# agiresearch/OpenP5

Measured on AMD Instinct MI355X. Metric: train_samples_per_sec, higher is better.
Workload: dtype bf16; 1 GPU; ML-1M-shaped sequential prompts, t5-small V=32100, B=64/GPU L=128 T=8, dropout 0.1, fwd+bwd+clip+AdamW (BASELINE.json configs[1]); global_batch=64, seq_len=128, tgt_len=8, parallelism=dp1

## Files before the change

openp5_amd/csrc/p5_attn.h:

```cpp
#pragma once
#include "p5_device.h"
#include "p5_rng.h"

struct P5AttnArgs {
  const void* Q; const void* K; const void* V;
  void* O;
  float* lse;
  const void* dO;
  void* dQ; void* dK; void* dV;
  float* Dvec;
  const float* rel_table;
  float* d_rel_table;
  const int* bucket_lut;
  int lut_half;
  const int64_t* kmask;
  int B, H, Lq, Lk;
  int ldq, ldk, ldv, ldo, lddo, lddq, lddk, lddv;
  int causal;
  int rel_copies;
  int rel_stride;
  P5Drop drop;
  uint32_t* keep_bits;
  float* dot_out;
};
// ... 992 lines not shown
#pragma unroll
          for (int t = 0; t < 4; ++t) {
            f32x4 sacc = {0.f, 0.f, 0.f, 0.f}, dpacc = {0.f, 0.f, 0.f, 0.f};
            mma16<T>(sacc, ld16(cK + t * 2048 + koff0), qf0);
            mma16<T>(sacc, ld16(cK + t * 2048 + koff1), qf1);
            mma16<T>(dpacc, ld16(cV + t * 2048 + koff0), dof0);
            mma16<T>(dpacc, ld16(cV + t * 2048 + koff1), dof1);
            const int kb = ch * 64 + t * 16 + g * 4;
            const f32x4 kn = *(const f32x4*)(skneg + kb);
            const float* pb = sbias + (kb - qic + a.Lq - 1);
            float mk[4] = {1.f, 1.f, 1.f, 1.f};
            if constexpr (MODE == 1) {
#pragma unroll
              for (int r = 0; r < 4; ++r) mk[r] = (kw[t][r] & lanebit) ? a.drop.scale : 0.f;
            } else if constexpr (MODE == 2) {
#pragma unroll
              for (int r = 0; r < 4; ++r) mk[r] = p5_keep(seed, a.drop.site_key, rowbase + (uint32_t)(kb + r), a.drop.thr) ? a.drop.scale : 0.f;
            }
#pragma unroll
            for (int r = 0; r < 4; ++r) {
              const int kj = kb + r;
              float ex = fmaf(sacc[r], P5_LOG2E, pb[r] + (kn[r] - lse_q));
              if constexpr (!PLAIN) ex = (qok & !(causal & (kj > qi))) ? ex : P5_NEG_INF;
              const float p = p5_exp2(ex);
              dsv[t][r] = p * (dpacc[r] * mk[r] - D_q);
            }
            if (do_rel) st4<T>(pw + li * DSTR + (DPAD + t * 16 + g * 4) * C::SZ, dsv[t]);
          }
        };
        if (use_bits) { if (plain) tiles(AttnBool<true>(), P5EpiTagA<1>()); else tiles(AttnBool<false>(), P5EpiTagA<1>()); }
        else if (do_drop) { if (plain) tiles(AttnBool<true>(), P5EpiTagA<2>()); else tiles(AttnBool<false>(), P5EpiTagA<2>()); }
        else { if (plain) tiles(AttnBool<true>(), P5EpiTagA<0>()); else tiles(AttnBool<false>(), P5EpiTagA<0>()); }
        if (do_rel) {
          P5_WAVE_SYNC();
          float x1 = 0.f, x2 = 0.f;
#pragma unroll
          for (int qr = 0; qr < 16; ++qr) {
            x1 += to_f<T>(*(const T*)(dg1 + qr * (DSTR + 2)));
            x2 += to_f<T>(*(const T*)(dg2 + qr * (DSTR + 2)));
          }
          x2 = lane < 15 ? x2 : 0.f;
          P5_WAVE_SYNC();
          const float y1 = __shfl(x1, src), y2 = __shfl(x2, src);
          R[ch] += up ? y1 : 0.f;
          R[ch + 1] += up ? y2 : y1;
          R[ch + 2] += up ? 0.f : y2;
        }
#pragma unroll
        for (int u = 0; u < 2; ++u) {
          const float d8[8] = {dsv[2 * u][0], dsv[2 * u][1], dsv[2 * u][2], dsv[2 * u][3], dsv[2 * u + 1][0], dsv[2 * u + 1][1], dsv[2 * u + 1][2], dsv[2 * u + 1][3]};
          const u32x4 da = pack16<T>(d8);
#pragma unroll
          for (int dt = 0; dt < 4; ++dt) {
            const char* base = cK + (u * 32 + trow) * 128 + (((dt * 2 + ((li >> 1) & 1)) ^ tsw) << 4) + (li & 1) * 8;
            const u32x2 lo = lds_tr16_b64(base);
            const u32x2 hi = lds_tr16_b64(base + 16 * 128);
            u32x4 kb4;
            kb4[0] = lo[0]; kb4[1] = lo[1]; kb4[2] = hi[0]; kb4[3] = hi[1];
            mma16<T>(dq[dt], da, kb4);
          }
        }
      }
    }
    const float one[4] = {1.f, 1.f, 1.f, 1.f};
    wave_store_16x64<T>((T*)a.dQ + (size_t)b * a.Lq * a.lddq + h * 64, a.lddq, q0, a.Lq, dq, one, pw, lane);
    if (do_rel && q0 + 128 < a.Lq) {
      P5_WAVE_SYNC();
      clear_diag_tile();
    }
    {
      const float t16 = R[16], t17 = R[17];
#pragma unroll
      for (int k = 17; k >= 2; --k) R[k] = R[k - 2];
      R[0] = t16; R[1] = t17;
    }
  }
  if (do_rel) {
    __syncthreads();
    float* rows = (float*)tKV;
    for (int i = lane; i < 1024; i += 64) rows[wave * 1024 + i] = 0.f;
    P5_WAVE_SYNC();
#pragma unroll
    for (int k = 0; k < 18; ++k) {
      int J = (cw - 2 * nblk + k) % 18;
      if (J < 0) J += 18;
      const int idx = 64 * J + lane - 16;
      if (idx >= 0 && idx < nrel) rows[wave * 1024 + idx] = R[k];
    }
    __syncthreads();
    for (int i = tid; i < nrel; i += NT) {
      float t = rows[i];
#pragma unroll
      for (int w = 1; w < 8; ++w) t += rows[w * 1024 + i];
      rows[i] = t;
    }
    __syncthreads();
    rel_bias_grad_flush<512>(a, h, b, rows, sbias, tid);
  }
}

template <int NQT>
__global__ __launch_bounds__(512) void p5_attn_bwd_dkv_head_kernel(P5AttnArgs a) {
  using T = bf16;
  using C = AttnC<T>;
  constexpr int LQ = NQT * 16, NT = 512, NP = LQ * 8 / NT;
  static_assert(NQT == 16 || NQT == 32, "whole-head attention backward: 256 or 512 query slots");
  __shared__ __attribute__((aligned(16))) char tQ[LQ * 128];
  __shared__ __attribute__((aligned(16))) char tDO[LQ * 128];
  __shared__ __attribute__((aligned(16))) char pbuf[8 * 16 * C::TS];
  constexpr int PADB = 64;
  __shared__ float sbias[PADB + 1024];
  __shared__ __attribute__((aligned(16))) float slse[LQ];
  __shared__ __attribute__((aligned(16))) float sD[LQ];

  const int tid = threadIdx.x, lane = tid & 63, wave = tid >> 6, g = lane >> 4, li = lane & 15;
  const int b = blockIdx.x / a.H, h = blockIdx.x % a.H;
  const T* Q = (const T*)a.Q + (size_t)b * a.Lq * a.ldq + h * 64;
  const T* K = (const T*)a.K + (size_t)b * a.Lk * a.ldk + h * 64;
  const T* V = (const T*)a.V + (size_t)b * a.Lk * a.ldv + h * 64;
  const T* dO = (const T*)a.dO + (size_t)b * a.Lq * a.lddo + h * 64;
  const int nrel = a.Lq + a.Lk - 1;
  {
    u32x4 rq[NP], rd[NP];
#pragma unroll
    for (int i = 0; i < NP; ++i) {
      const int p = tid + i * NT, row = p >> 3, pc = p & 7;
      rq[i] = row < a.Lq ? ld16(Q + (size_t)row * a.ldq + pc * 8) : zero16();
    }
#pragma unroll
    for (int i = 0; i < NP; ++i) {
      const int p = tid + i * NT, row = p >> 3, pc = p & 7;
      rd[i] = row < a.Lq ? ld16(dO + (size_t)row * a.lddo + pc * 8) : zero16();
    }
    for (int i = tid; i < PADB + 1023; i += NT) {
      const int j = i - PADB;
      sbias[i] = (a.rel_table && j >= 0 && j < nrel) ? P5_LOG2E * a.rel_table[a.bucket_lut[j - (a.Lq - 1) + a.lut_half] * a.H + h] : 0.f;
    }
    for (int i = tid; i < LQ; i += NT) {
      slse[i] = i < a.Lq ? P5_LOG2E * attn_bwd_row_lse(a.lse[((size_t)b * a.H + h) * a.Lq + i]) : 0.f;
      sD[i] = i < a.Lq ? a.Dvec[((size_t)b * a.H + h) * a.Lq + i] : 0.f;
    }
#pragma unroll
    for (int i = 0; i < NP; ++i) {
      const int p = tid + i * NT, row = p >> 3, pc = p & 7;
      st16(tQ + row * 128 + ((pc ^ ((row >> 1) & 7)) << 4), rq[i]);
      st16(tDO + row * 128 + ((pc ^ ((row >> 1) & 7)) << 4), rd[i]);
    }
  }
  u32x4 kn[2], vn[2];
  bool kok_n;
  {
    const int krow = wave * 16 + li;
#pragma unroll
    for (int c = 0; c < 2; ++c) {
      kn[c] = krow < a.Lk ? ld16(K + (size_t)krow * a.ldk + c * 32 + g * 8) : zero16();
      vn[c] = krow < a.Lk ? ld16(V + (size_t)krow * a.ldv + c * 32 + g * 8) : zero16();
    }
    kok_n = krow < a.Lk && (!a.kmask || a.kmask[(size_t)b * a.Lk + krow] != 0);
  }
  __syncthreads();

  const bool causal = a.causal != 0;
  const bool do_drop = a.drop.state != nullptr && a.drop.thr != 0;
  const bool use_bits = do_drop && a.keep_bits != nullptr;
  const uint32_t seed = p5_seed(a.drop);
  const int ksw = (li >> 1) & 7;
  const int koff0 = li * 128 + (((0 + g) ^ ksw) << 4), koff1 = li * 128 + (((4 + g) ^ ksw) << 4);
  const int trow = g * 4 + (li >> 2), tsw = (g * 2 + (li >> 3)) & 7;
  char* pw = pbuf + wave * 16 * C::TS;
  const int nqc = (a.Lq + 63) / 64;
  for (int k0 = wave * 16; k0 < a.Lk; k0 += 128) {
    const u32x4 kf0 = kn[0], kf1 = kn[1], vf0 = vn[0], vf1 = vn[1];
    const bool kok = kok_n;
    const int kj = k0 + li;
    if (k0 + 128 < a.Lk) {
      const int krow = k0 + 128 + li;
#pragma unroll
      for (int c = 0; c < 2; ++c) {
        kn[c] = krow < a.Lk ? ld16(K + (size_t)krow * a.ldk + c * 32 + g * 8) : zero16();
        vn[c] = krow < a.Lk ? ld16(V + (size_t)krow * a.ldv + c * 32 + g * 8) : zero16();
      }
      kok_n = krow < a.Lk && (!a.kmask || a.kmask[(size_t)b * a.Lk + krow] != 0);
    }
    const uint32_t headbase = (uint32_t)((((size_t)b * a.H + h) * a.Lq) * a.Lk) + (uint32_t)kj;
    const char* kpk = use_bits ? (const char*)(a.keep_bits + ((size_t)b * a.H + h) * ((a.Lq + 15) / 16) * 256) +
                                     ((((kj >> 3) & 1) * 128 + (kj >> 4) * 4 + (kj & 3)) * 4 + ((kj >> 2) & 1) * 2) : nullptr;
    f32x4 dk[4], dv[4];
#pragma unroll
    for (int dt = 0; dt < 4; ++dt) { dk[dt] = (f32x4){0.f, 0.f, 0.f, 0.f}; dv[dt] = (f32x4){0.f, 0.f, 0.f, 0.f}; }
    unsigned pcn[4] = {0u, 0u, 0u, 0u};
    if (use_bits) {
#pragma unroll
      for (int t = 0; t < 4; ++t) pcn[t] = t * 16 < a.Lq ? *(const unsigned short*)(kpk + (size_t)t * 1024) : 0u;
    }
    for (int qc = 0; qc < nqc; ++qc) {
      const char* cQ = tQ + qc * 64 * 128;
      const char* cD = tDO + qc * 64 * 128;
      float pv[4][4], dsv[4][4];
      const unsigned pcc[4] = {pcn[0], pcn[1], pcn[2], pcn[3]};
      if (use_bits && (qc + 1) * 64 < a.Lq) {
#pragma unroll
        for (int t = 0; t < 4; ++t) pcn[t] = ((qc + 1) * 4 + t) * 16 < a.Lq ? *(const unsigned short*)(kpk + (size_t)((qc + 1) * 4 + t) * 1024) : 0u;
      }
      const bool plain = !causal && (qc + 1) * 64 <= a.Lq;
      auto tiles = [&](auto plain_c, auto mode_c) {
        constexpr bool PLAIN = decltype(plain_c)::value;
        constexpr int MODE = decltype(mode_c)::value;
#pragma unroll
        for (int t = 0; t < 4; ++t) {
          f32x4 sacc = {0.f, 0.f, 0.f, 0.f}, dpacc = {0.f, 0.f, 0.f, 0.f};
          mma16<T>(sacc, ld16(cQ + t * 2048 + koff0), kf0);
          mma16<T>(sacc, ld16(cQ + t * 2048 + koff1), kf1);
          mma16<T>(dpacc, ld16(cD + t * 2048 + koff0), vf0);
          mma16<T>(dpacc, ld16(cD + t * 2048 + koff1), vf1);
          const int qb = qc * 64 + t * 16 + g * 4;
          const f32x4 ls = *(const f32x4*)(slse + qb), dd = *(const f32x4*)(sD + qb);
          const float* pbq = sbias + (PADB + kj - qb + a.Lq - 4);
          const float bias[4] = {pbq[3], pbq[2], pbq[1], pbq[0]};
          const uint32_t tbase = headbase + (uint32_t)qb * (uint32_t)a.Lk;
          float mk[4] = {1.f, 1.f, 1.f, 1.f};
          if constexpr (MODE == 1) {
            const unsigned piece = pcc[t] >> (g * 4);
#pragma unroll
            for (int r = 0; r < 4; ++r) mk[r] = ((piece >> r) & 1u) ? a.drop.scale : 0.f;
          } else if constexpr (MODE == 2) {
#pragma unroll
            for (int r = 0; r < 4; ++r) mk[r] = p5_keep(seed, a.drop.site_key, tbase + (uint32_t)r * (uint32_t)a.Lk, a.drop.thr) ? a.drop.scale : 0.f;
          }
#pragma unroll
          for (int r = 0; r < 4; ++r) {
            const int qi = qb + r;
            const bool ok = PLAIN ? kok : (kok & (qi < a.Lq) & !(causal & (kj > qi)));
            float ex = fmaf(sacc[r], P5_LOG2E, bias[r] - ls[r]);
            ex = ok ? ex : P5_NEG_INF;
            const float p = p5_exp2(ex);
            pv[t][r] = p * mk[r];
            dsv[t][r] = p * (dpacc[r] * mk[r] - dd[r]);
          }
        }
      };
      if (use_bits) { if (plain) tiles(AttnBool<true>(), P5EpiTagA<1>()); else tiles(AttnBool<false>(), P5EpiTagA<1>()); }
      else if (do_drop) { if (plain) tiles(AttnBool<true>(), P5EpiTagA<2>()); else tiles(AttnBool<false>(), P5EpiTagA<2>()); }
      else { if (plain) tiles(AttnBool<true>(), P5EpiTagA<0>()); else tiles(AttnBool<false>(), P5EpiTagA<0>()); }
#pragma unroll
      for (int u = 0; u < 2; ++u) {
        const float p8[8] = {pv[2 * u][0], pv[2 * u][1], pv[2 * u][2], pv[2 * u][3], pv[2 * u + 1][0], pv[2 * u + 1][1], pv[2 * u + 1][2], pv[2 * u + 1][3]};
        const float d8[8] = {dsv[2 * u][0], dsv[2 * u][1], dsv[2 * u][2], dsv[2 * u][3], dsv[2 * u + 1][0], dsv[2 * u + 1][1], dsv[2 * u + 1][2], dsv[2 * u + 1][3]};
        const u32x4 pa = pack16<T>(p8), sa = pack16<T>(d8);
#pragma unroll
        for (int dt = 0; dt < 4; ++dt) {
          const int off = (u * 32 + trow) * 128 + (((dt * 2 + ((li >> 1) & 1)) ^ tsw) << 4) + (li & 1) * 8;
          u32x2 lo = lds_tr16_b64(cD + off), hi = lds_tr16_b64(cD + off + 16 * 128);
          u32x4 f;
          f[0] = lo[0]; f[1] = lo[1]; f[2] = hi[0]; f[3] = hi[1];
          mma16<T>(dv[dt], pa, f);
          lo = lds_tr16_b64(cQ + off);
          hi = lds_tr16_b64(cQ + off + 16 * 128);
          f[0] = lo[0]; f[1] = lo[1]; f[2] = hi[0]; f[3] = hi[1];
          mma16<T>(dk[dt], sa, f);
        }
      }
    }
    const float one[4] = {1.f, 1.f, 1.f, 1.f};
    wave_store_16x64<T>((T*)a.dK + (size_t)b * a.Lk * a.lddk + h * 64, a.lddk, k0, a.Lk, dk, one, pw, lane);
    wave_store_16x64<T>((T*)a.dV + (size_t)b * a.Lk * a.lddv + h * 64, a.lddv, k0, a.Lk, dv, one, pw, lane);
  }
}

#ifdef P5_EMU
#define P5_ATTN_SMALL_OCC
#else
#define P5_ATTN_SMALL_OCC __attribute__((amdgpu_waves_per_eu(2, 2)))
#endif
template <class T>
__global__ __launch_bounds__(256) P5_ATTN_SMALL_OCC void p5_attn_bwd_small_kernel(P5AttnArgs a) {
  using C = AttnC<T>;
  constexpr int KR = C::KCH;
  constexpr int RS = 64 + 16;
    __shared__ __attribute__((aligned(16))) char tileKV[2 * 64 * C::TS];
  char* const tileK = tileKV;
  char* const tileV = tileKV + 64 * C::TS; __shared__ __attribute__((aligned(16))) char tileQ[32 * C::TS];
  __shared__ __attribute__((aligned(16))) char tileDO[32 * C::TS];
  __shared__ __attribute__((aligned(16))) char aP[4][16 * RS];
  __shared__ __attribute__((aligned(16))) char aS[4][16 * RS];
  __shared__ __attribute__((aligned(16))) char bS[4][16 * RS];
  __shared__ __attribute__((aligned(16))) char wscr[4][16 * C::TS];
  static_assert(2 * 64 * C::TS >= 4 * 16 * 68 * 4, "the dQ partial sums reuse the K and V tiles");
  float (*sdq)[16][68] = (float (*)[16][68])tileKV;
  __shared__ __attribute__((aligned(16))) float sbias[1024];
  __shared__ float sdb[4][528];
  __shared__ __attribute__((aligned(16))) float slse[16];
  __shared__ __attribute__((aligned(16))) float sD[16];

  const int tid = threadIdx.x, lane = tid & 63, wave = tid >> 6, g = lane >> 4, li = lane & 15;
  const int b = blockIdx.y / a.H, h = blockIdx.y % a.H;
  const T* Q = (const T*)a.Q + (size_t)b * a.Lq * a.ldq + h * 64;
  const T* K = (const T*)a.K + (size_t)b * a.Lk * a.ldk + h * 64;
  const T* V = (const T*)a.V + (size_t)b * a.Lk * a.ldv + h * 64;
  const T* dO = (const T*)a.dO + (size_t)b * a.Lq * a.lddo + h * 64;
  const T* O = (const T*)a.O + (size_t)b * a.Lq * a.ldo + h * 64;
  const int nrel = a.Lq + a.Lk - 1;
  const int nch = (a.Lk + 63) / 64;

  for (int p = tid; p < 32 * C::PPR; p += 256) {
    const int row = p / C::PPR, pc = p % C::PPR;
    st16(tileQ + row * C::TS + pc * 16, row < a.Lq ? ld16(Q + (size_t)row * a.ldq + pc * C::EPF) : zero16());
    st16(tileDO + row * C::TS + pc * 16, row < a.Lq ? ld16(dO + (size_t)row * a.lddo + pc * C::EPF) : zero16());
  }
  if (a.rel_table) {
    for (int i = tid; i < nrel; i += 256) sbias[i] = a.rel_table[a.bucket_lut[i - (a.Lq - 1) + a.lut_half] * a.H + h];
    if (a.d_rel_table)
      for (int i = tid; i < 4 * 528; i += 256) (&sdb[0][0])[i] = 0.f;
  }
  if (tid < 64) {
    const int q = tid >> 2, part = tid & 3;
    float d = 0.f;
    if (q < a.Lq) {
      for (int c = 0; c < 16; c += C::EPF) {
        float x[8], y[8];
        unpack16<T>(ld16(dO + (size_t)q * a.lddo + part * 16 + c), x);
        unpack16<T>(ld16(O + (size_t)q * a.ldo + part * 16 + c), y);
#pragma unroll
        for (int e = 0; e < C::EPF; ++e) d += x[e] * y[e];
      }
    }
    d += __shfl_xor(d, 1);
    d += __shfl_xor(d, 2);
    if (part == 0) {
      sD[q] = d;
      slse[q] = q < a.Lq ? a.lse[((size_t)b * a.H + h) * a.Lq + q] : 0.f;
      if (a.Dvec && q < a.Lq) a.Dvec[((size_t)b * a.H + h) * a.Lq + q] = d;
    }
  }
  for (int i = lane; i < 16 * RS / 4; i += 64) {
    ((unsigned*)aP[wave])[i] = 0u; ((unsigned*)aS[wave])[i] = 0u; ((unsigned*)bS[wave])[i] = 0u;
  }
  __syncthreads();

  u32x4 qf[C::NCK], dof[C::NCK];
#pragma unroll
  for (int c = 0; c < C::NCK; ++c) { qf[c] = tile_frag_kc<T>(tileQ, 0, c, lane); dof[c] = tile_frag_kc<T>(tileDO, 0, c, lane); }
  const bool causal = a.causal != 0;
  const bool do_drop = a.drop.state != nullptr && a.drop.thr != 0;
  const uint32_t seed = p5_seed(a.drop);
  const int qb = g * 4;
  const f32x4 ls = *(const f32x4*)(slse + qb), dd = *(const f32x4*)(sD + qb);
  const int kc_w = (wave * 16) / KR, koff = (wave * 16) % KR;

  f32x4 dq[4];
#pragma unroll
  for (int dt = 0; dt < 4; ++dt) dq[dt] = (f32x4){0.f, 0.f, 0.f, 0.f};

  for (int ch = 0; ch < nch; ++ch) {
    __syncthreads();
    stage_tile64<T>(tileK, K + (size_t)ch * 64 * a.ldk, a.ldk, a.Lk - ch * 64, tid);
    stage_tile64<T>(tileV, V + (size_t)ch * 64 * a.ldv, a.ldv, a.Lk - ch * 64, tid);
    __syncthreads();
    const int k0 = ch * 64 + wave * 16, kj = k0 + li;
    if (k0 < a.Lk) {
      const bool kok = kj < a.Lk && (!a.kmask || a.kmask[(size_t)b * a.Lk + kj] != 0);
      f32x4 sacc = {0.f, 0.f, 0.f, 0.f}, dpacc = {0.f, 0.f, 0.f, 0.f};
#pragma unroll
      for (int c = 0; c < C::NCK; ++c) {
        mma16<T>(sacc, qf[c], tile_frag_kc<T>(tileK, wave * 16, c, lane));
        mma16<T>(dpacc, dof[c], tile_frag_kc<T>(tileV, wave * 16, c, lane));
      }
      float pv[4], dsv[4];
#pragma unroll
      for (int r = 0; r < 4; ++r) {
        const int qi = qb + r;
        const int qic = qi < a.Lq ? qi : a.Lq - 1;
        const float bias = a.rel_table ? sbias[(kj < a.Lk ? kj : a.Lk - 1) - qic + a.Lq - 1] : 0.f;
        const float mk = do_drop ? (p5_keep(seed, a.drop.site_key, (uint32_t)((((size_t)b * a.H + h) * a.Lq + qic) * a.Lk) + (uint32_t)kj, a.drop.thr) ? a.drop.scale : 0.f) : 1.f;
        const bool ok = kok & (qi < a.Lq) & !(causal & (kj > qi));
        const float p = p5_exp<T>((sacc[r] + bias) - ls[r]);
        pv[r] = ok ? p * mk : 0.f;
        dsv[r] = ok ? p * (dpacc[r] * mk - dd[r]) : 0.f;
      }
      P5_WAVE_SYNC();
      st4<T>(aP[wave] + li * RS + qb * C::SZ, pv);
      st4<T>(aS[wave] + li * RS + qb * C::SZ, dsv);
#pragma unroll
      for (int r = 0; r < 4; ++r) *(T*)(bS[wave] + (qb + r) * RS + (koff + li) * C::SZ) = from_f<T>(dsv[r]);
      P5_WAVE_SYNC();
      if (a.d_rel_table) {
        for (int dg = lane; dg < 31; dg += 64) {
          float sum = 0.f;
#pragma unroll
          for (int qr = 0; qr < 16; ++qr) {
            const int kcol = dg - 15 + qr;
            if (kcol >= 0 && kcol < 16) sum += to_f<T>(*(const T*)(bS[wave] + qr * RS + (koff + kcol) * C::SZ));
          }
          const int idx = k0 + dg - 15 + a.Lq - 1;
          if (idx >= 0 && idx < nrel) sdb[wave][idx] += sum;
        }
      }
      f32x4 dk[4], dv[4];
      const u32x4 pa = ld16(aP[wave] + li * RS + g * 16), sa = ld16(aS[wave] + li * RS + g * 16);
      const u32x4 dsa = ld16(bS[wave] + li * RS + g * 16);
#pragma unroll
      for (int dt = 0; dt < 4; ++dt) {
        dk[dt] = (f32x4){0.f, 0.f, 0.f, 0.f}; dv[dt] = (f32x4){0.f, 0.f, 0.f, 0.f};
        mma16<T>(dv[dt], pa, tile_frag_ks<T>(tileDO, dt * 16, 0, lane));
        mma16<T>(dk[dt], sa, tile_frag_ks<T>(tileQ, dt * 16, 0, lane));
        mma16<T>(dq[dt], dsa, tile_frag_ks<T>(tileK, dt * 16, kc_w, lane));
      }
      const float one[4] = {1.f, 1.f, 1.f, 1.f};
      wave_store_16x64<T>((T*)a.dK + (size_t)b * a.Lk * a.lddk + h * 64, a.lddk, k0, a.Lk, dk, one, wscr[wave], lane);
      wave_store_16x64<T>((T*)a.dV + (size_t)b * a.Lk * a.lddv + h * 64, a.lddv, k0, a.Lk, dv, one, wscr[wave], lane);
    }
  }
  __syncthreads();
#pragma unroll
  for (int dt = 0; dt < 4; ++dt)
#pragma unroll
    for (int r = 0; r < 4; ++r) sdq[wave][g * 4 + r][dt * 16 + li] = dq[dt][r];
  __syncthreads();
  if (wave == 0) {
    f32x4 t[4];
#pragma unroll
    for (int dt = 0; dt < 4; ++dt)
#pragma unroll
      for (int r = 0; r < 4; ++r)
        t[dt][r] = ((sdq[0][g * 4 + r][dt * 16 + li] + sdq[1][g * 4 + r][dt * 16 + li]) + sdq[2][g * 4 + r][dt * 16 + li]) + sdq[3][g * 4 + r][dt * 16 + li];
    const float one[4] = {1.f, 1.f, 1.f, 1.f};
    wave_store_16x64<T>((T*)a.dQ + (size_t)b * a.Lq * a.lddq + h * 64, a.lddq, 0, a.Lq, t, one, wscr[0], lane);
  }
  if (a.d_rel_table) {
    for (int i = tid; i < nrel; i += 256) sdb[0][i] = ((sdb[0][i] + sdb[1][i]) + sdb[2][i]) + sdb[3][i];
    __syncthreads();
    rel_bias_grad_flush<256>(a, h, b, &sdb[0][0], sbias, tid);
  }
}

__device__ static __forceinline__ u32x4 frag_ks_stride(const char* lds, int stride, int e0, int kc, int lane) {
  const int g = lane >> 4, i = lane & 15;
  const char* base = lds + (kc * 32 + g * 8 + (i >> 2)) * stride + (e0 + (i & 3) * 4) * 2;
  const u32x2 lo = lds_tr16_b64(base), hi = lds_tr16_b64(base + 4 * stride);
  u32x4 r;
  r[0] = lo[0]; r[1] = lo[1]; r[2] = hi[0]; r[3] = hi[1];
  return r;
}

template <class T>
__global__ __launch_bounds__(512) void p5_attn_bwd_fused_kernel(P5AttnArgs a) {
  static_assert(sizeof(T) == 2, "fused attention backward: bf16 only");
  using C = AttnC<T>;
  constexpr int TP = 128 * 2 + 16;
  __shared__ __attribute__((aligned(16))) char tK[128 * C::TS];
  __shared__ __attribute__((aligned(16))) char tV[128 * C::TS];
  __shared__ __attribute__((aligned(16))) char tQ[128 * C::TS];
  __shared__ __attribute__((aligned(16))) char tDO[128 * C::TS];
  __shared__ __attribute__((aligned(16))) char mP[128 * TP];
  __shared__ __attribute__((aligned(16))) char mS[128 * TP];
  __shared__ float sbias[256];
  __shared__ float sdiag[8 * 144];
  __shared__ __attribute__((aligned(16))) float skneg[128];

  const int tid = threadIdx.x, lane = tid & 63, wave = tid >> 6, g = lane >> 4, li = lane & 15;
  const int b = blockIdx.x / a.H, h = blockIdx.x % a.H;
  const T* Q = (const T*)a.Q + (size_t)b * a.Lq * a.ldq + h * 64;
  const T* K = (const T*)a.K + (size_t)b * a.Lk * a.ldk + h * 64;
  const T* V = (const T*)a.V + (size_t)b * a.Lk * a.ldv + h * 64;
  const T* dO = (const T*)a.dO + (size_t)b * a.Lq * a.lddo + h * 64;
  const T* O = (const T*)a.O + (size_t)b * a.Lq * a.ldo + h * 64;
  const int nrel = a.Lq + a.Lk - 1;

  u32x4 rq[2], rk[2], rv[2], rdo[2], of[2];
#pragma unroll
  for (int i = 0; i < 2; ++i) {
    const int p = tid + i * 512, row = p >> 3, pc = p & 7;
    rq[i] = row < a.Lq ? ld16(Q + (size_t)row * a.ldq + pc * 8) : zero16();
    rdo[i] = row < a.Lq ? ld16(dO + (size_t)row * a.lddo + pc * 8) : zero16();
    rk[i] = row < a.Lk ? ld16(K + (size_t)row * a.ldk + pc * 8) : zero16();
    rv[i] = row < a.Lk ? ld16(V + (size_t)row * a.ldv + pc * 8) : zero16();
  }
  const int q0 = wave * 16, qi = q0 + li;
  const bool qok = qi < a.Lq;
  const int qic = qok ? qi : a.Lq - 1;
#pragma unroll
  for (int c = 0; c < 2; ++c) of[c] = qok ? ld16(O + (size_t)qi * a.ldo + c * 32 + g * 8) : zero16();
  const float lse_q = qok ? P5_LOG2E * attn_bwd_row_lse(a.lse[((size_t)b * a.H + h) * a.Lq + qi]) : 0.f;
  stage_bias_mask(a, b, h, sbias, skneg, 128, tid, P5_LOG2E, 256);
#pragma unroll
  for (int i = 0; i < 2; ++i) {
    const int p = tid + i * 512, row = p >> 3, pc = p & 7;
    st16(tQ + row * C::TS + pc * 16, rq[i]);
    st16(tDO + row * C::TS + pc * 16, rdo[i]);
    st16(tK + row * C::TS + pc * 16, rk[i]);
    st16(tV + row * C::TS + pc * 16, rv[i]);
  }
  __syncthreads();

  const bool causal = a.causal != 0;
  const bool do_drop = a.drop.state != nullptr && a.drop.thr != 0;
  const uint32_t seed = p5_seed(a.drop);
  const uint32_t rowbase = (uint32_t)((((size_t)b * a.H + h) * a.Lq + qi) * a.Lk);
  u32x4 qf[2], dof[2];
  float D_q = 0.f;
#pragma unroll
  for (int c = 0; c < 2; ++c) {
    qf[c] = tile_frag_kc<T>(tQ, q0, c, lane);
    dof[c] = tile_frag_kc<T>(tDO, q0, c, lane);
    float x[8], y[8];
    unpack16<T>(dof[c], x);
    unpack16<T>(of[c], y);
#pragma unroll
    for (int e = 0; e < 8; ++e) D_q += x[e] * y[e];
  }
  D_q += __shfl_xor(D_q, 16);
  D_q += __shfl_xor(D_q, 32);
  char* myP = mP + qi * TP;
  char* myS = mS + qi * TP;
  const bool plain = !causal && q0 + 16 <= a.Lq;
#pragma unroll
  for (int t = 0; t < 8; ++t) {
    f32x4 sacc = {0.f, 0.f, 0.f, 0.f}, dpacc = {0.f, 0.f, 0.f, 0.f};
#pragma unroll
    for (int c = 0; c < 2; ++c) {
      mma16<T>(sacc, tile_frag_kc<T>(tK, t * 16, c, lane), qf[c]);
      mma16<T>(dpacc, tile_frag_kc<T>(tV, t * 16, c, lane), dof[c]);
    }
    const int kb = t * 16 + g * 4;
    const f32x4 kn = *(const f32x4*)(skneg + kb);
    const float* pb = sbias + (kb - qic + a.Lq - 1);
    float mk[4] = {1.f, 1.f, 1.f, 1.f};
    if (do_drop) {
#pragma unroll
      for (int r = 0; r < 4; ++r) mk[r] = p5_keep(seed, a.drop.site_key, rowbase + (uint32_t)(kb + r), a.drop.thr) ? a.drop.scale : 0.f;
    }
    float pv[4], dsv[4];
#pragma unroll
    for (int r = 0; r < 4; ++r) {
      const int kj = kb + r;
      float ex = fmaf(sacc[r], P5_LOG2E, pb[r] + (kn[r] - lse_q));
      if (!plain) ex = (qok & !(causal & (kj > qi))) ? ex : P5_NEG_INF;
      const float p = p5_exp2(ex);
      pv[r] = p * mk[r];
      dsv[r] = p * (dpacc[r] * mk[r] - D_q);
    }
    st4<T>(myP + kb * 2, pv);
    st4<T>(myS + kb * 2, dsv);
  }
  P5_WAVE_SYNC();
  if (a.d_rel_table) {
    for (int dd = lane; dd < 128 + 15; dd += 64) {
      float sum = 0.f;
#pragma unroll
      for (int qr = 0; qr < 16; ++qr) {
        const int kcol = dd - 15 + qr;
        const bool in = (kcol >= 0) & (kcol < 128);
        const float v = to_f<T>(*(const T*)(mS + (q0 + qr) * TP + (in ? kcol : 0) * 2));
        sum += in ? v : 0.f;
      }
      sdiag[wave * 144 + dd] = sum;
    }
  }
  f32x4 dq[4];
#pragma unroll
  for (int dt = 0; dt < 4; ++dt) dq[dt] = (f32x4){0.f, 0.f, 0.f, 0.f};
#pragma unroll
  for (int kc = 0; kc < 4; ++kc) {
    const u32x4 dsa = ld16(myS + kc * 64 + g * 16);
#pragma unroll
    for (int dt = 0; dt < 4; ++dt) mma16<T>(dq[dt], dsa, tile_frag_ks<T>(tK, dt * 16, kc, lane));
  }
  __syncthreads();

  if (a.d_rel_table) {
    float pv[4];
    int pb[4];
#pragma unroll
    for (int j = 0; j < 4; ++j) {
      const int i = lane + 64 * j;
      float v = 0.f;
      pb[j] = -1;
      if (i < nrel) {
        pb[j] = a.bucket_lut[i - (a.Lq - 1) + a.lut_half] & 63;
#pragma unroll
        for (int w = 0; w < 8; ++w) {
          const int dd = i + 15 + 16 * w - (a.Lq - 1);
          const bool in = (dd >= 0) & (dd < 128 + 15);
          const float x = sdiag[w * 144 + (in ? dd : 0)];
          v += in ? x : 0.f;
        }
      }
      pv[j] = v;
    }
    for (int bk = wave; bk < a.rel_copies; bk += 8) {
      float acc = 0.f;
#pragma unroll
      for (int j = 0; j < 4; ++j) acc += pb[j] == bk ? pv[j] : 0.f;
      acc = wave_sum(acc);
      if (lane == 0) a.d_rel_table[(size_t)b * a.rel_stride + bk * a.H + h] = acc;
    }
  }
  const float one[4] = {1.f, 1.f, 1.f, 1.f};
  char* scratch = tK + wave * 16 * C::TS;
  const bool want_dot = a.dot_out != nullptr;
  float dot[2] = {0.f, 0.f};
  u32x4 fwk[2], fwq[2], fwv[2];
  if (want_dot) {
#pragma unroll
    for (int p = 0; p < 2; ++p) {
      const int off = (wave * 16 + p * 8 + (lane >> 3)) * C::TS + (lane & 7) * 16;
      fwk[p] = ld16(tK + off);
      fwq[p] = ld16(tQ + off);
      fwv[p] = ld16(tV + off);
    }
    wave_store_16x64_dot<T>((T*)a.dQ + (size_t)b * a.Lq * a.lddq + h * 64, a.lddq, q0, a.Lq, dq, scratch, lane, fwq, dot);
  } else {
    wave_store_16x64<T>((T*)a.dQ + (size_t)b * a.Lq * a.lddq + h * 64, a.lddq, q0, a.Lq, dq, one, scratch, lane);
  }

  const int k0 = wave * 16;
  f32x4 dk[4], dv[4];
#pragma unroll
  for (int dt = 0; dt < 4; ++dt) { dk[dt] = (f32x4){0.f, 0.f, 0.f, 0.f}; dv[dt] = (f32x4){0.f, 0.f, 0.f, 0.f}; }
#pragma unroll
  for (int kc = 0; kc < 4; ++kc) {
    const u32x4 pa = frag_ks_stride(mP, TP, k0, kc, lane);
    const u32x4 sa = frag_ks_stride(mS, TP, k0, kc, lane);
#pragma unroll
    for (int dt = 0; dt < 4; ++dt) {
      mma16<T>(dv[dt], pa, tile_frag_ks<T>(tDO, dt * 16, kc, lane));
      mma16<T>(dk[dt], sa, tile_frag_ks<T>(tQ, dt * 16, kc, lane));
    }
  }
  if (want_dot) {
    wave_store_16x64_dot<T>((T*)a.dK + (size_t)b * a.Lk * a.lddk + h * 64, a.lddk, k0, a.Lk, dk, scratch, lane, fwk, dot);
    wave_store_16x64_dot<T>((T*)a.dV + (size_t)b * a.Lk * a.lddv + h * 64, a.lddv, k0, a.Lk, dv, scratch, lane, fwv, dot);
#pragma unroll
    for (int p = 0; p < 2; ++p) {
      float t = dot[p];
      t += __shfl_xor(t, 1);
      t += __shfl_xor(t, 2);
      t += __shfl_xor(t, 4);
      const int tok = wave * 16 + p * 8 + (lane >> 3);
      if ((lane & 7) == 0 && tok < a.Lq) a.dot_out[((size_t)b * a.Lq + tok) * a.H + h] = t;
    }
    return;
  }
  wave_store_16x64<T>((T*)a.dK + (size_t)b * a.Lk * a.lddk + h * 64, a.lddk, k0, a.Lk, dk, one, scratch, lane);
  wave_store_16x64<T>((T*)a.dV + (size_t)b * a.Lk * a.lddv + h * 64, a.lddv, k0, a.Lk, dv, one, scratch, lane);
}
```

Measured before the change: 16250 samples/s.

## Prefetch K/V chunks into registers and batch prologue loads in attention backward

For 16-bit types, the attention backward kernel now issues all prologue global loads (Q, dO, O, lse, bucket LUT, rel bias, first K/V chunk) into registers before any shared-memory stores, using scheduling fences to group them. It also software-pipelines the K/V chunk loop, fetching chunk ch+1 into registers while chunk ch is computed, and reads the key mask together with that fetch. This is meant to hide global-memory latency in a short kernel (Lk=128, few chunks). The cost is higher register pressure, which could lower occupancy.

```diff
diff --git a/openp5_amd/csrc/p5_attn.h b/openp5_amd/csrc/p5_attn.h
--- a/openp5_amd/csrc/p5_attn.h
+++ b/openp5_amd/csrc/p5_attn.h
@@ -1318,34 +1318,133 @@
   const int nrel = a.Lq + a.Lk - 1;
   const int nch = (a.Lk + 63) / 64;
 
-  for (int p = tid; p < 32 * C::PPR; p += 256) {
-    const int row = p / C::PPR, pc = p % C::PPR;
-    st16(tileQ + row * C::TS + pc * 16, row < a.Lq ? ld16(Q + (size_t)row * a.ldq + pc * C::EPF) : zero16());
-    st16(tileDO + row * C::TS + pc * 16, row < a.Lq ? ld16(dO + (size_t)row * a.lddo + pc * C::EPF) : zero16());
-  }
-  if (a.rel_table) {
-    for (int i = tid; i < nrel; i += 256) sbias[i] = a.rel_table[a.bucket_lut[i - (a.Lq - 1) + a.lut_half] * a.H + h];
-    if (a.d_rel_table)
-      for (int i = tid; i < 4 * 528; i += 256) (&sdb[0][0])[i] = 0.f;
-  }
-  if (tid < 64) {
+  constexpr int NPKV = 64 * C::PPR / 256, NREL = 3;
+  constexpr bool PRE = sizeof(T) == 2;
+  u32x4 rk[NPKV], rv[NPKV];
+  const int64_t* const kmp = a.kmask ? a.kmask + (size_t)b * a.Lk : (const int64_t*)a.Q;
+  int64_t rkm = 1;
+  auto kv_fetch = [&](int ch) {
+    const int valid_rows = a.Lk - ch * 64;
+#pragma unroll
+    for (int i = 0; i < NPKV; ++i) {
+      const int p = tid + i * 256, row = p / C::PPR, pc = p % C::PPR;
+      const int rowc = row < valid_rows ? row : valid_rows - 1;
+      rk[i] = ld16(K + ((size_t)ch * 64 + rowc) * a.ldk + pc * C::EPF);
+      rv[i] = ld16(V + ((size_t)ch * 64 + rowc) * a.ldv + pc * C::EPF);
+    }
+    const int kj = ch * 64 + wave * 16 + li;
+    rkm = kmp[(a.kmask && kj < a.Lk) ? kj : 0];
+  };
+  auto kv_publish = [&](int ch) {
+    const int valid_rows = a.Lk - ch * 64;
+#pragma unroll
+    for (int i = 0; i < NPKV; ++i) {
+      const int p = tid + i * 256, row = p / C::PPR, pc = p % C::PPR;
+      st16(tileK + row * C::TS + pc * 16, row < valid_rows ? rk[i] : zero16());
+      st16(tileV + row * C::TS + pc * 16, row < valid_rows ? rv[i] : zero16());
+    }
+  };
+
+  if constexpr (PRE) {
+    constexpr int NQ = 32 * C::PPR / 256, ND = 16 / C::EPF;
+    const bool has_tab = a.rel_table != nullptr;
+    const int* const lutp = has_tab ? a.bucket_lut : (const int*)a.lse;
+    const float* const tab = has_tab ? a.rel_table : a.lse;
+    const int tab_ld = has_tab ? a.H : 0, tab_h = has_tab ? h : 0, lut0 = has_tab ? a.lut_half - (a.Lq - 1) : 0;
+    int lutv[NREL];
+#pragma unroll
+    for (int j = 0; j < NREL; ++j) {
+      const int i = tid + j * 256;
+      lutv[j] = lutp[lut0 + ((has_tab && i < nrel) ? i : 0)];
+    }
+    P5_SCHED_FENCE();
+    kv_fetch(0);
+    u32x4 tq[NQ], tdo[NQ], xd[ND], yo[ND];
+#pragma unroll
+    for (int i = 0; i < NQ; ++i) {
+      const int p = tid + i * 256, row = p / C::PPR, pc = p % C::PPR;
+      const int rowc = row < a.Lq ? row : a.Lq - 1;
+      tq[i] = ld16(Q + (size_t)rowc * a.ldq + pc * C::EPF);
+      tdo[i] = ld16(dO + (size_t)rowc * a.lddo + pc * C::EPF);
+    }
     const int q = tid >> 2, part = tid & 3;
-    float d = 0.f;
-    if (q < a.Lq) {
-      for (int c = 0; c < 16; c += C::EPF) {
-        float x[8], y[8];
-        unpack16<T>(ld16(dO + (size_t)q * a.lddo + part * 16 + c), x);
-        unpack16<T>(ld16(O + (size_t)q * a.ldo + part * 16 + c), y);
-#pragma unroll
-        for (int e = 0; e < C::EPF; ++e) d += x[e] * y[e];
-      }
-    }
-    d += __shfl_xor(d, 1);
-    d += __shfl_xor(d, 2);
-    if (part == 0) {
-      sD[q] = d;
-      slse[q] = q < a.Lq ? a.lse[((size_t)b * a.H + h) * a.Lq + q] : 0.f;
-      if (a.Dvec && q < a.Lq) a.Dvec[((size_t)b * a.H + h) * a.Lq + q] = d;
+    const int qc = q < a.Lq ? q : a.Lq - 1;
+#pragma unroll
+    for (int k = 0; k < ND; ++k) {
+      xd[k] = ld16(dO + (size_t)qc * a.lddo + part * 16 + k * C::EPF);
+      yo[k] = ld16(O + (size_t)qc * a.ldo + part * 16 + k * C::EPF);
+    }
+    const float lse_r = a.lse[((size_t)b * a.H + h) * a.Lq + qc];
+    P5_SCHED_FENCE();
+    float tb[NREL];
+#pragma unroll
+    for (int j = 0; j < NREL; ++j) tb[j] = tab[lutv[j] * tab_ld + tab_h];
+    P5_SCHED_FENCE();
+#pragma unroll
+    for (int i = 0; i < NQ; ++i) {
+      const int p = tid + i * 256, row = p / C::PPR, pc = p % C::PPR;
+      st16(tileQ + row * C::TS + pc * 16, row < a.Lq ? tq[i] : zero16());
+      st16(tileDO + row * C::TS + pc * 16, row < a.Lq ? tdo[i] : zero16());
+    }
+    if (has_tab) {
+#pragma unroll
+      for (int j = 0; j < NREL; ++j) {
+        const int i = tid + j * 256;
+        if (i < nrel) sbias[i] = tb[j];
+      }
+      if (a.d_rel_table)
+        for (int i = tid; i < 4 * 528; i += 256) (&sdb[0][0])[i] = 0.f;
+    }
+    if (tid < 64) {
+      float d = 0.f;
+      if (q < a.Lq) {
+#pragma unroll
+        for (int k = 0; k < ND; ++k) {
+          float x[8], y[8];
+          unpack16<T>(xd[k], x);
+          unpack16<T>(yo[k], y);
+#pragma unroll
+          for (int e = 0; e < C::EPF; ++e) d += x[e] * y[e];
+        }
+      }
+      d += __shfl_xor(d, 1);
+      d += __shfl_xor(d, 2);
+      if (part == 0) {
+        sD[q] = d;
+        slse[q] = q < a.Lq ? lse_r : 0.f;
+        if (a.Dvec && q < a.Lq) a.Dvec[((size_t)b * a.H + h) * a.Lq + q] = d;
+      }
+    }
+  } else {
+    for (int p = tid; p < 32 * C::PPR; p += 256) {
+      const int row = p / C::PPR, pc = p % C::PPR;
+      st16(tileQ + row * C::TS + pc * 16, row < a.Lq ? ld16(Q + (size_t)row * a.ldq + pc * C::EPF) : zero16());
+      st16(tileDO + row * C::TS + pc * 16, row < a.Lq ? ld16(dO + (size_t)row * a.lddo + pc * C::EPF) : zero16());
+    }
+    if (a.rel_table) {
+      for (int i = tid; i < nrel; i += 256) sbias[i] = a.rel_table[a.bucket_lut[i - (a.Lq - 1) + a.lut_half] * a.H + h];
+      if (a.d_rel_table)
+        for (int i = tid; i < 4 * 528; i += 256) (&sdb[0][0])[i] = 0.f;
+    }
+    if (tid < 64) {
+      const int q = tid >> 2, part = tid & 3;
+      float d = 0.f;
+      if (q < a.Lq) {
+        for (int c = 0; c < 16; c += C::EPF) {
+          float x[8], y[8];
+          unpack16<T>(ld16(dO + (size_t)q * a.lddo + part * 16 + c), x);
+          unpack16<T>(ld16(O + (size_t)q * a.ldo + part * 16 + c), y);
+#pragma unroll
+          for (int e = 0; e < C::EPF; ++e) d += x[e] * y[e];
+        }
+      }
+      d += __shfl_xor(d, 1);
+      d += __shfl_xor(d, 2);
+      if (part == 0) {
+        sD[q] = d;
+        slse[q] = q < a.Lq ? a.lse[((size_t)b * a.H + h) * a.Lq + q] : 0.f;
+        if (a.Dvec && q < a.Lq) a.Dvec[((size_t)b * a.H + h) * a.Lq + q] = d;
+      }
     }
   }
   for (int i = lane; i < 16 * RS / 4; i += 64) {
@@ -1369,12 +1468,13 @@
 
   for (int ch = 0; ch < nch; ++ch) {
     __syncthreads();
-    stage_tile64<T>(tileK, K + (size_t)ch * 64 * a.ldk, a.ldk, a.Lk - ch * 64, tid);
-    stage_tile64<T>(tileV, V + (size_t)ch * 64 * a.ldv, a.ldv, a.Lk - ch * 64, tid);
+    if constexpr (!PRE) kv_fetch(ch);
+    kv_publish(ch);
+    const bool kok = ch * 64 + wave * 16 + li < a.Lk && (!a.kmask || rkm != 0);
     __syncthreads();
+    if constexpr (PRE) { if (ch + 1 < nch) kv_fetch(ch + 1); }
     const int k0 = ch * 64 + wave * 16, kj = k0 + li;
     if (k0 < a.Lk) {
-      const bool kok = kj < a.Lk && (!a.kmask || a.kmask[(size_t)b * a.Lk + kj] != 0);
       f32x4 sacc = {0.f, 0.f, 0.f, 0.f}, dpacc = {0.f, 0.f, 0.f, 0.f};
 #pragma unroll
       for (int c = 0; c < C::NCK; ++c) {
```

New measurement: 16350 samples/s, median of 6. No clear change (+0.6%).
